# apple/ml-pgdvs

Hardware: AMD Instinct MI355X
Metric: novel-view frames/s at 1080p x 24 src frames; achieved HBM GB/s vs gfx950 peak (higher is better)
Workload: dtype f32

## Files before the change

### ml-pgdvs_amd/csrc/common.h

```cpp
#pragma once
#include <hip/hip_runtime.h>
#include <stdint.h>
#include <stdio.h>

#include "../../include/pgdvs_hip.h"

#define PGDVS_API extern "C" __attribute__((visibility("default")))

namespace pgdvs {

void set_error(const char *fmt, ...);

struct Options {
  int agg_ordered;
  int agg_stage;
  int gnt_fp32;
  int knn_no_tpq;
  int knn_stats;
  float raster_bound_density;
  int side_thread;
};
const char *last_error_text();
int option_int(const int &field);
float option_float(const float &field);
const Options &options();

inline hipStream_t as_stream(pgdvs_stream_t s) { return reinterpret_cast<hipStream_t>(s); }

inline int check_launch(const char *what) {
  hipError_t e = hipGetLastError();
  if (e != hipSuccess) {
    set_error("%s: %s", what, hipGetErrorString(e));
    return PGDVS_ERR_LAUNCH;
  }
  return PGDVS_OK;
}

bool prof_enabled();
void prof_begin(const char *name, hipStream_t s);
void prof_end(hipStream_t s);
struct ProfScope {
  hipStream_t s;
  bool on;
  ProfScope(const char *name, hipStream_t st) : s(st), on(prof_enabled()) {
    if (on) prof_begin(name, s);
  }
  ~ProfScope() {
    if (on) prof_end(s);
  }
};

#define PGDVS_LAUNCH(name, kernel, grid, block, lds, stream, ...)       \
  do {                                                                   \
    pgdvs::ProfScope _ps(name, stream);                                  \
    hipLaunchKernelGGL(kernel, grid, block, lds, stream, __VA_ARGS__);   \
  } while (0)

#define PGDVS_REQUIRE(cond, ...)      \
  do {                                \
    if (!(cond)) {                    \
      pgdvs::set_error(__VA_ARGS__);  \
      return PGDVS_ERR_INVALID;       \
    }                                 \
  } while (0)

constexpr int kWave = 64;

__global__ static void __launch_bounds__(256) fill_bytes_kernel(uint4 *__restrict__ p, int64_t n16, uint32_t v32) {
  const uint4 v = make_uint4(v32, v32, v32, v32);
  for (int64_t i = (int64_t)blockIdx.x * blockDim.x + threadIdx.x; i < n16; i += (int64_t)gridDim.x * blockDim.x) p[i] = v;
}

inline hipError_t fill_async(void *ptr, unsigned char byte, size_t nbytes, hipStream_t st) {
  if (nbytes < (1u << 20) || (reinterpret_cast<uintptr_t>(ptr) & 15) != 0) return hipMemsetAsync(ptr, byte, nbytes, st);
  const int64_t n16 = (int64_t)(nbytes / 16);
  const uint32_t v32 = 0x01010101u * byte;
  const unsigned grid = (unsigned)((n16 + 255) / 256 < 4096 ? (n16 + 255) / 256 : 4096);
  {
    ProfScope ps("fill_bytes", st);
    hipLaunchKernelGGL(fill_bytes_kernel, dim3(grid), dim3(256), 0, st, reinterpret_cast<uint4 *>(ptr), n16, v32);
  }
  const size_t tail = nbytes - (size_t)n16 * 16;
  if (tail) return hipMemsetAsync(static_cast<char *>(ptr) + (size_t)n16 * 16, byte, tail, st);
  return hipGetLastError();
}

inline int64_t cdiv(int64_t a, int64_t b) { return (a + b - 1) / b; }
inline int64_t align_up(int64_t a, int64_t b) { return cdiv(a, b) * b; }

struct Carver {
  char *base;
  int64_t off = 0;
  template <class T>
  T *take(int64_t bytes, int64_t align = 256) {
    T *p = reinterpret_cast<T *>(base + off);
    off += align_up(bytes, align);
    return p;
  }
};

struct CamBlock {
  float v[PGDVS_CAM_BLOCK];
};

__host__ __device__ inline int inv_f64(const double *a, double *out, int n) {
  double m[4][8];
  for (int i = 0; i < n; ++i) {
    for (int j = 0; j < n; ++j) {
      m[i][j] = a[i * n + j];
      m[i][n + j] = (i == j) ? 1.0 : 0.0;
    }
  }
  for (int c = 0; c < n; ++c) {
    int piv = c;
    double best = fabs(m[c][c]);
    for (int r = c + 1; r < n; ++r) {
      double v = fabs(m[r][c]);
      if (v > best) {
        best = v;
        piv = r;
      }
    }
    if (best == 0.0) return -1;
    if (piv != c) {
      for (int j = 0; j < 2 * n; ++j) {
        double t = m[c][j];
        m[c][j] = m[piv][j];
        m[piv][j] = t;
      }
    }
    double d = m[c][c];
    for (int j = 0; j < 2 * n; ++j) m[c][j] = m[c][j] / d;
    for (int r = 0; r < n; ++r) {
      if (r == c) continue;
      double f = m[r][c];
      if (f == 0.0) continue;
      for (int j = 0; j < 2 * n; ++j) m[r][j] = m[r][j] - f * m[c][j];
    }
  }
  for (int i = 0; i < n; ++i)
    for (int j = 0; j < n; ++j) out[i * n + j] = m[i][n + j];
  return 0;
}

__host__ __device__ inline int cam_block_from_flat(const float *flat_cam, float *blk) {
  const float *K = flat_cam + 2;
  const float *c2w = flat_cam + 18;
  double k3[9], k3i[9], c4[16], c4i[16];
  for (int i = 0; i < 3; ++i)
    for (int j = 0; j < 3; ++j) k3[i * 3 + j] = (double)K[i * 4 + j];
  for (int i = 0; i < 16; ++i) c4[i] = (double)c2w[i];
  int bad = 0;
  if (inv_f64(k3, k3i, 3) != 0) bad = 1;
  if (inv_f64(c4, c4i, 4) != 0) bad = 1;
  float kinv[9], w2c[16];
  for (int i = 0; i < 9; ++i) kinv[i] = bad ? __builtin_nanf("") : (float)k3i[i];
  for (int i = 0; i < 16; ++i) w2c[i] = bad ? __builtin_nanf("") : (float)c4i[i];
  for (int i = 0; i < 9; ++i) blk[PGDVS_CAM_KINV + i] = kinv[i];
  for (int i = 0; i < 3; ++i) {
    for (int j = 0; j < 3; ++j) {
      float s = c2w[i * 4 + 0] * kinv[0 * 3 + j];
      s = s + c2w[i * 4 + 1] * kinv[1 * 3 + j];
      s = s + c2w[i * 4 + 2] * kinv[2 * 3 + j];
      blk[PGDVS_CAM_M + i * 3 + j] = s;
      blk[PGDVS_CAM_R + i * 3 + j] = c2w[i * 4 + j];
    }
    blk[PGDVS_CAM_O + i] = c2w[i * 4 + 3];
// ... 54 lines not shown
```

### ml-pgdvs_amd/csrc/error.cpp

```cpp
#include <hip/hip_runtime.h>
#include <stdarg.h>
#include <string.h>

#include <map>
#include <mutex>
#include <string>
#include <vector>
#include <stdio.h>

#include <stdlib.h>

#include "common.h"

namespace pgdvs {
static thread_local char g_err[512] = "";

void set_error(const char *fmt, ...) {
  va_list ap;
  va_start(ap, fmt);
  vsnprintf(g_err, sizeof(g_err), fmt, ap);
  va_end(ap);
}

const char *last_error_text() { return g_err; }

struct ProfRec {
  const char *name;
  hipEvent_t a, b;
};
static std::mutex g_prof_mu;
static bool g_prof_on = false;
static std::vector<ProfRec> g_prof_recs;
static std::vector<hipEvent_t> g_prof_pool;
static thread_local ProfRec g_prof_cur;

bool prof_enabled() { return g_prof_on; }

static hipEvent_t prof_event() {
  std::lock_guard<std::mutex> lk(g_prof_mu);
  if (!g_prof_pool.empty()) {
    hipEvent_t e = g_prof_pool.back();
    g_prof_pool.pop_back();
    return e;
  }
  hipEvent_t e;
  (void)hipEventCreate(&e);
  return e;
}

void prof_begin(const char *name, hipStream_t s) {
  g_prof_cur.name = name;
  g_prof_cur.a = prof_event();
  g_prof_cur.b = prof_event();
  (void)hipEventRecord(g_prof_cur.a, s);
}

void prof_end(hipStream_t s) {
  (void)hipEventRecord(g_prof_cur.b, s);
  std::lock_guard<std::mutex> lk(g_prof_mu);
  g_prof_recs.push_back(g_prof_cur);
}
}

namespace pgdvs {
static Options options_from_env() {
  auto flag = [](const char *name) {
    const char *v = getenv(name);
    return v != nullptr && v[0] == '1' ? 1 : 0;
  };
  Options o;
  o.agg_ordered = flag("PGDVS_AGG_ORDERED");
  o.agg_stage = getenv("PGDVS_AGG_STAGE") != nullptr && getenv("PGDVS_AGG_STAGE")[0] == '0' ? 0 : 1;
  o.gnt_fp32 = flag("PGDVS_GNT_FP32");
  o.knn_no_tpq = flag("PGDVS_KNN_NO_TPQ");
  o.knn_stats = flag("PGDVS_KNN_STATS");
  const char *d = getenv("PGDVS_RASTER_BOUND_DENSITY");
  o.raster_bound_density = d != nullptr ? (float)atof(d) : 2.2f;
  o.side_thread = getenv("PGDVS_SIDE_THREAD") != nullptr && getenv("PGDVS_SIDE_THREAD")[0] == '0' ? 0 : 1;
  return o;
}
static Options g_options = options_from_env();
const Options &options() { return g_options; }
int option_int(const int &field) { return __atomic_load_n(&field, __ATOMIC_RELAXED); }
float option_float(const float &field) {
  float v;
  __atomic_load(&field, &v, __ATOMIC_RELAXED);
  return v;
}
struct OptionName {
  const char *name;
  int *i;
  float *f;
};
static const OptionName kOptionNames[] = {
    {"agg_ordered", &g_options.agg_ordered, nullptr},   {"agg_stage", &g_options.agg_stage, nullptr},
    {"gnt_fp32", &g_options.gnt_fp32, nullptr},
    {"knn_no_tpq", &g_options.knn_no_tpq, nullptr},     {"knn_stats", &g_options.knn_stats, nullptr},
    {"raster_bound_density", nullptr, &g_options.raster_bound_density},
    {"side_thread", &g_options.side_thread, nullptr},
};
}

extern "C" __attribute__((visibility("default"))) int pgdvs_option_set(const char *name, double value) {
  for (const auto &o : pgdvs::kOptionNames) {
    if (name != nullptr && strcmp(name, o.name) == 0) {
      if (o.i != nullptr) {
        __atomic_store_n(o.i, value != 0.0 ? 1 : 0, __ATOMIC_RELAXED);
      } else {
        float v = (float)value;
        __atomic_store(o.f, &v, __ATOMIC_RELAXED);
      }
      return PGDVS_OK;
    }
  }
  pgdvs::set_error("pgdvs_option_set: unknown option '%s'", name ? name : "(null)");
  return PGDVS_ERR_INVALID;
}

extern "C" __attribute__((visibility("default"))) double pgdvs_option_get(const char *name) {
  for (const auto &o : pgdvs::kOptionNames) {
    if (name != nullptr && strcmp(name, o.name) == 0)
      return o.i != nullptr ? (double)pgdvs::option_int(*o.i) : (double)pgdvs::option_float(*o.f);
  }
  return __builtin_nan("");
}

namespace pgdvs {
__global__ void prof_null_kernel() {}

static double prof_bracket_overhead_ms() {
  static double cached = -1.0;
  if (cached >= 0.0) return cached;
  hipEvent_t a, b;
  if (hipEventCreate(&a) != hipSuccess || hipEventCreate(&b) != hipSuccess) return 0.0;
  double best = 1e30;
  (void)hipDeviceSynchronize();
  for (int i = 0; i < 32; ++i) {
    (void)hipEventRecord(a, nullptr);
    prof_null_kernel<<<1, 64, 0, nullptr>>>();
    (void)hipEventRecord(b, nullptr);
    (void)hipEventSynchronize(b);
    float ms = 0.f;
    if (hipEventElapsedTime(&ms, a, b) == hipSuccess && ms > 0.f && ms < best) best = ms;
  }
  (void)hipEventDestroy(a);
  (void)hipEventDestroy(b);
  cached = best < 1e29 ? best : 0.0;
  return cached;
}
}

extern "C" __attribute__((visibility("default"))) double pgdvs_prof_overhead_ms(void) {
  return pgdvs::prof_bracket_overhead_ms();
}

extern "C" __attribute__((visibility("default"))) void pgdvs_prof_enable(int on) {
  std::lock_guard<std::mutex> lk(pgdvs::g_prof_mu);
  pgdvs::g_prof_on = on != 0;
}

extern "C" __attribute__((visibility("default"))) int pgdvs_prof_report(char *buf, int buf_len) {
  using namespace pgdvs;
  std::vector<ProfRec> recs;
  {
    std::lock_guard<std::mutex> lk(g_prof_mu);
    recs.swap(g_prof_recs);
  }
  std::map<std::string, std::pair<int, double>> agg;
  const double overhead = recs.empty() ? 0.0 : prof_bracket_overhead_ms();
  for (auto &r : recs) {
    (void)hipEventSynchronize(r.b);
    float ms = 0.f;
    (void)hipEventElapsedTime(&ms, r.a, r.b);
    auto &e = agg[r.name];
    e.first += 1;
    e.second += ms > overhead ? ms - overhead : 0.0;
    std::lock_guard<std::mutex> lk(g_prof_mu);
    g_prof_pool.push_back(r.a);
    g_prof_pool.push_back(r.b);
  }
  std::string out;
  for (auto &kv : agg) {
    char line[256];
    snprintf(line, sizeof(line), "%s %d %.6f\n", kv.first.c_str(), kv.second.first, kv.second.second);
    out += line;
  }
  if (buf && buf_len > 0) {
    strncpy(buf, out.c_str(), (size_t)buf_len - 1);
    buf[buf_len - 1] = 0;
  }
  return (int)agg.size();
}

extern "C" __attribute__((visibility("default"))) const char *pgdvs_last_error(void) {
  return pgdvs::g_err;
}
extern "C" __attribute__((visibility("default"))) int pgdvs_abi_version(void) { return 1; }
extern "C" __attribute__((visibility("default"))) const char *pgdvs_build_arch(void) {
  return "gfx950";
}
```

### ml-pgdvs_amd/csrc/static_agg.hip

```cpp
#include <cmath>
#include <vector>

#include "common.h"
#include "wave.h"

namespace pgdvs {

struct ProjF64 {
  double K3[9];
  double w2c[16];
  int affine;
  int ksparse;
  double M[12];
  double tol_scale;
  int screen;
  float M32[12];
  float e32[3];
  int screen32;
};

__device__ __forceinline__ double refined_rcp(double b) {
  double r = __builtin_amdgcn_rcp(b);
  double e = __builtin_fma(-b, r, 1.0);
  r = __builtin_fma(r, e, r);
  e = __builtin_fma(-b, r, 1.0);
  return __builtin_fma(r, e, r);
}

__device__ __forceinline__ bool trunc_div_in_range(double a, double b, double r, int hi, int &out) {
  double q = a * r;
  double f = floor(q);
  double dist = fmin(q - f, (f + 1.0) - q);
  if (!(dist > fabs(q) * 1e-13 + 1e-290)) q = a / b;
  if (!(q >= 0.0 && q <= (double)hi)) return false;
  out = (int)q;
  return true;
}

constexpr int kProjChunk = 10;
struct ProjChunk {
  ProjF64 p[kProjChunk];
};
static_assert(sizeof(ProjChunk) + 64 <= 4096, "agg_params_kernel's arguments");

struct PushConsts;
__global__ void agg_params_kernel(ProjChunk c, ProjF64 *__restrict__ dst, float *__restrict__ pc32, int first, int n, float q_hi) {
  const int words = (int)(sizeof(ProjF64) / 4);
  for (int k = threadIdx.x; k < n * words; k += blockDim.x)
    reinterpret_cast<uint32_t *>(dst + first)[k] = reinterpret_cast<const uint32_t *>(&c.p[0])[k];
  for (int k = threadIdx.x; k < n * 16; k += blockDim.x) {
    const ProjF64 &pj = c.p[k >> 4];
    const int j = k & 15;
    float v = 0.0f;
    if (j < 12) {
      v = pj.M32[j];
    } else if (!pj.screen32) {
      v = j < 15 ? INFINITY : 0.0f;
    } else if (j == 12) {
      const double e01 = pj.e32[0] > pj.e32[1] ? (double)pj.e32[0] : (double)pj.e32[1];
      v = (float)((e01 + ((double)q_hi + 1.0) * (double)pj.e32[2]) * 1.001 * 1.000001);
    } else if (j == 13) {
      v = (float)(((double)q_hi * 2.6e-7 + 1e-7) * 1.000001);
    } else if (j == 14) {
      v = (float)((0.125 - ((double)q_hi * 2.6e-7 + 1e-7) * 1.000001) * 0.999999);
    }
    pc32[(size_t)(first + (k >> 4)) * 16 + j] = v;
  }
}

struct ByteStamp {
  uint8_t *occ_all;
  int64_t P;
  unsigned *stat;
  __device__ __forceinline__ void operator()(int f, int q) const { (occ_all + (int64_t)f * P)[(unsigned)q] = 1; }
};
template <class Stamp>
__device__ __attribute__((noinline)) void mark_reference_order(const ProjF64 *__restrict__ pj, double x, double y,
                                                               double z, int H, int W, int f, const Stamp &stamp) {
  double vc[4];
#pragma unroll
  for (int k = 0; k < 3; ++k) {
    double s = pj->w2c[k * 4 + 0] * x;
    s = s + pj->w2c[k * 4 + 1] * y;
    s = s + pj->w2c[k * 4 + 2] * z;
    s = s + pj->w2c[k * 4 + 3];
    vc[k] = s;
  }
  double cx = vc[0], cy = vc[1], cz = vc[2];
  if (!pj->affine) {
    double s = pj->w2c[12] * x;
    s = s + pj->w2c[13] * y;
    s = s + pj->w2c[14] * z;
    s = s + pj->w2c[15];
    cx = vc[0] / s;
    cy = vc[1] / s;
    cz = vc[2] / s;
  }
  double pp[3];
  if (pj->ksparse) {
    pp[0] = pj->K3[0] * cx + pj->K3[2] * cz;
    pp[1] = pj->K3[4] * cy + pj->K3[5] * cz;
    pp[2] = cz;
  } else {
#pragma unroll
    for (int k = 0; k < 3; ++k) {
      double s = pj->K3[k * 3 + 0] * cx;
      s = s + pj->K3[k * 3 + 1] * cy;
      s = s + pj->K3[k * 3 + 2] * cz;
      pp[k] = s;
    }
  }
  int row, col;
  const double rz = refined_rcp(pp[2]);
  if (!trunc_div_in_range(pp[1], pp[2], rz, H - 1, row)) return;
  if (!trunc_div_in_range(pp[0], pp[2], rz, W - 1, col)) return;
  stamp(f, row * W + col);
}

template <class Stamp>
__device__ __attribute__((noinline)) void mark_fp64(const ProjF64 *__restrict__ pj, float xf, float yf, float zf, int H,
                                                    int W, int f, const Stamp &stamp) {
  const double x = (double)xf, y = (double)yf, z = (double)zf;
  if (pj->screen) {
    const double *M = pj->M;
    const double amax = fmax(fmax(fabs(x), fabs(y)), fmax(fabs(z), 1.0));
    const double s0 = __builtin_fma(M[0], x, __builtin_fma(M[1], y, __builtin_fma(M[2], z, M[3])));
    const double s1 = __builtin_fma(M[4], x, __builtin_fma(M[5], y, __builtin_fma(M[6], z, M[7])));
    const double s2 = __builtin_fma(M[8], x, __builtin_fma(M[9], y, __builtin_fma(M[10], z, M[11])));
    const double r = refined_rcp(s2);
    const double qx = s0 * r, qy = s1 * r;
    const double tol = pj->tol_scale * amax * fabs(r);
    const double fx = floor(qx), fy = floor(qy);
    const double dx = fmin(qx - fx, (fx + 1.0) - qx), dy = fmin(qy - fy, (fy + 1.0) - qy);
    if (dx > tol * (1.0 + fabs(qx)) && dy > tol * (1.0 + fabs(qy))) {
      if (qy >= 0.0 && qy <= (double)(H - 1) && qx >= 0.0 && qx <= (double)(W - 1)) stamp(f, (int)qy * W + (int)qx);
      return;
    }
  }
  atomicAdd(stamp.stat, 1u);
  mark_reference_order(pj, x, y, z, H, W, f, stamp);
}

typedef float f2v __attribute__((ext_vector_type(2)));
struct PushConsts {
  float M[12];
  float e[3];
  float pad;
};
static_assert(sizeof(PushConsts) == 64, "PushConsts");

struct AppendSrc {
  const float *depth;
  const float *rgb;
  float *cloud;
  float *xyz;
  int P, W;
};
struct f3 { float x, y, z; };

__device__ __forceinline__ f3 append_row(const AppendSrc &a, const CamBlock &cam, int p, int64_t pos, bool write,
                                         float d_in = __builtin_nanf(""), float *d_out = nullptr, const f3 *c_in = nullptr) {
  int r, col;
  if (a.P < (1 << 24)) {
    r = (int)(((float)p + 0.5f) * (1.0f / (float)a.W));
    col = p - r * a.W;
    if (col < 0) {
      --r;
      col += a.W;
    } else if (col >= a.W) {
      ++r;
      col -= a.W;
    }
  } else {
    r = p / a.W;
    col = p - r * a.W;
  }
  const float u = (float)col, v = (float)r;
  const float d = d_in == d_in ? d_in : a.depth[p];
  if (d_out) *d_out = d;
  float X[3];
#pragma unroll
  for (int ax = 0; ax < 3; ++ax) {
    float dir = cam.v[PGDVS_CAM_M + ax * 3 + 0] * u;
    dir = dir + cam.v[PGDVS_CAM_M + ax * 3 + 1] * v;
    dir = dir + cam.v[PGDVS_CAM_M + ax * 3 + 2];
    X[ax] = cam.v[PGDVS_CAM_O + ax] + dir * d;
  }
  f3 xq;
  xq.x = X[0];
  xq.y = X[1];
  xq.z = X[2];
  if (write) {
    const f3 c = c_in ? *c_in : *reinterpret_cast<const f3 *>(a.rgb + (size_t)p * 3);
    float2 *o = reinterpret_cast<float2 *>(a.cloud + pos * 6);
    o[0] = make_float2(X[0], X[1]);
    o[1] = make_float2(X[2], c.x);
    o[2] = make_float2(c.y, c.z);
    *reinterpret_cast<f3 *>(a.xyz + pos * 3) = xq;
  }
  return xq;
}

constexpr int kSelThreads = 512;
constexpr int kSelItems = 16;
constexpr int kSelTile = kSelThreads * kSelItems;
constexpr int kPushThreads = 256;
constexpr int kPushQueue = 1024;
constexpr int kPushQueueSmall = 512;
constexpr int kPushMaxFpg = 32;

template <class Stamp, class Rec>
__device__ __forceinline__ unsigned screen_frames(const Rec &rec, const int fa, const int fb,
                                                  const bool live, float x, float y, float z, const float wm1,
                                                  const float hm1, const int W, const Stamp &stamp) {
  if (!live) x = y = z = __builtin_nanf("");
  const float amax = fmaxf(fmaxf(fabsf(x), fabsf(y)), fmaxf(fabsf(z), 1.0f));
  unsigned dmask = 0;
  auto frame = [&](const int f, const PushConsts &c) {
    const float *M = c.M;
    const f2v p0 = {M[0], M[1]}, p1 = {M[2], M[3]}, p2 = {M[4], M[5]}, p3 = {M[6], M[7]};
    const f2v xx = {x, x}, yy = {y, y}, zz = {z, z};
    const f2v s01 = __builtin_elementwise_fma(p0, xx, __builtin_elementwise_fma(p1, yy, __builtin_elementwise_fma(p2, zz, p3)));
    const float s0 = s01.x, s1 = s01.y;
    const float s2 = __builtin_fmaf(M[8], x, __builtin_fmaf(M[9], y, __builtin_fmaf(M[10], z, M[11])));
    const float r = __builtin_amdgcn_rcpf(s2);
    const float qx = s0 * r, qy = s1 * r;
    const float u = c.e[0] * (fabsf(r) * amax);
    const float gx = __builtin_amdgcn_fractf(qx), gy = __builtin_amdgcn_fractf(qy);
    const float dx = fminf(gx, 1.0f - gx), dy = fminf(gy, 1.0f - gy);
    const bool sure = (__builtin_fmaf(qx + qy, 0.0f, u) < c.e[2]) & (fabsf(s2) < 0x1p100f);
    const bool clear = fminf(dx, dy) - u > c.e[1];
    const float mi = fminf(fminf(qx, wm1 - qx), fminf(qy, hm1 - qy));
    if (sure & clear & (mi >= 0.0f)) stamp(f, (int)qy * W + (int)qx);
    dmask |= ((sure & (clear | (mi < -0.5f))) ? 0u : 1u) << (f - fa);
  };
  PushConsts ca = rec(fa);
  for (int f = fa; f < fb; f += 2) {
    const PushConsts cb = rec(f + 1);
    frame(f, ca);
    if (f + 1 < fb) {
      ca = rec(f + 2);
      frame(f + 1, cb);
    }
  }
  return live ? dmask : 0u;
}

constexpr int kAggStatWords = 65;
template <int kQueue, int kThreads, class Stamp>
__device__ __forceinline__ void queue_doubtful(uint4 *s_q, int *s_qn, const unsigned dmask, const float x, const float y,
                                               const float z, const int fa, const bool last,
                                               const ProjF64 *__restrict__ proj, const int H, const int W, const Stamp &stamp) {
  if (dmask != 0) {
    const int slot = atomicAdd(s_qn, 1);
    if (slot < kQueue) {
      s_q[slot] = make_uint4(__float_as_uint(x), __float_as_uint(y), __float_as_uint(z), dmask);
    } else {
      atomicAdd(stamp.stat + 1 + (blockIdx.x & 63), 1u);
      for (unsigned m = dmask; m; m &= m - 1) {
        const int f = fa + __builtin_ctz(m);
        mark_fp64(proj + f, x, y, z, H, W, f, stamp);
      }
    }
  }
  __syncthreads();
  const int qn = *s_qn < kQueue ? *s_qn : kQueue;
  __syncthreads();
  if (last || qn + kThreads > kQueue) {
    if (threadIdx.x == 0) s_qn[1] += qn;
    for (int e = threadIdx.x; e < qn; e += kThreads) {
      const uint4 q = s_q[e];
      const float px = __uint_as_float(q.x), py = __uint_as_float(q.y), pz = __uint_as_float(q.z);
      for (unsigned m = q.w; m; m &= m - 1) {
        const int f = fa + __builtin_ctz(m);
        mark_fp64(proj + f, px, py, pz, H, W, f, stamp);
      }
    }
    __syncthreads();
    if (threadIdx.x == 0) {
      *s_qn = 0;
      if (last && s_qn[1] > 0) {
        atomicAdd(stamp.stat + 1 + (blockIdx.x & 63), (unsigned)s_qn[1]);
        s_qn[1] = 0;
      }
    }
    __syncthreads();
  }
}

template <int kQueue>
__global__ void __launch_bounds__(kPushThreads)
agg_push_kernel(const float *__restrict__ xyz, const int64_t *__restrict__ cnts, int src,
                const ProjF64 *__restrict__ proj, const PushConsts *__restrict__ pc, int f_lo, int f_hi, int fpg, int H, int W,
                uint8_t *__restrict__ occ_all, const int32_t *__restrict__ sel_pix, AppendSrc app, CamBlock cam,
                unsigned *__restrict__ stat) {
  __shared__ uint4 s_q[kQueue];
  __shared__ int s_qn[2];
  const int64_t begin = cnts[src], end = cnts[src + 1];
  if (begin >= end) return;
  const ByteStamp stamp{occ_all, (int64_t)H * W, stat};
  const float wm1 = (float)(W - 1), hm1 = (float)(H - 1);
  if (threadIdx.x == 0) s_qn[0] = s_qn[1] = 0;
  __syncthreads();
  bool first_iter = true;
  for (int fa = f_lo + (int)blockIdx.y * fpg; fa < f_hi || (first_iter && sel_pix != nullptr && blockIdx.y == 0);
       fa += (int)gridDim.y * fpg, first_iter = false) {
  const int fb = fa >= f_hi ? fa : (fa + fpg < f_hi ? fa + fpg : f_hi);
  const int64_t n_chunks = (end - begin + kPushThreads - 1) / kPushThreads;
  const int64_t per_xcd = (n_chunks + 7) / 8;
  const int64_t c_lo = (int64_t)(blockIdx.x & 7) * per_xcd;
  const int64_t c_hi = c_lo + per_xcd < n_chunks ? c_lo + per_xcd : n_chunks;
  const int64_t c_step = gridDim.x >> 3 ? gridDim.x >> 3 : 1;
  for (int64_t ch = c_lo + (int64_t)(blockIdx.x >> 3); ch < c_hi; ch += c_step) {
    const int64_t i = begin + ch * kPushThreads + threadIdx.x;
    const bool live = i < end;
    float x = 0.f, y = 0.f, z = 0.f;
    if (live && sel_pix != nullptr) {
      const f3 X = append_row(app, cam, sel_pix[i - begin], i, blockIdx.y == 0 && first_iter);
      x = X.x;
      y = X.y;
      z = X.z;
    } else if (live) {
      x = xyz[i * 3 + 0];
      y = xyz[i * 3 + 1];
      z = xyz[i * 3 + 2];
    }
    unsigned dmask = 0;
    if (fa < fb) dmask = screen_frames([pc](const int f) { return pc[f]; }, fa, fb, live, x, y, z, wm1, hm1, W, stamp);
    queue_doubtful<kQueue, kPushThreads>(s_q, s_qn, dmask, x, y, z, fa, ch + c_step >= c_hi, proj, H, W, stamp);
  }
  }
}


constexpr int kBitTileWords = kSelTile / 32;
constexpr int kStepThreads = 256;
constexpr int kStepPx = 16;
constexpr int kStepChunkPx = 128;
constexpr int kStepChunks = kStepThreads * kStepPx / kStepChunkPx;

__device__ __forceinline__ int64_t step_chunk_of(const int b, const int r, const int gx) {
  const int L = gx >> 3, xcd = b & 7, l = b >> 3;
  const int j = r * L + l;
  return ((int64_t)(j / kStepChunks) * 8 + xcd) * kStepChunks + (j % kStepChunks);
}
__device__ __forceinline__ void step_owner_of(const int64_t g, const int gx, int &b, int &r) {
  const int L = gx >> 3;
  const int64_t stripe = g / kStepChunks;
  const int xcd = (int)(stripe & 7);
  const int j = (int)(stripe >> 3) * kStepChunks + (int)(g % kStepChunks);
  r = j / L;
  b = (j - r * L) * 8 + xcd;
}

constexpr unsigned kSelSpinLimit = 1u << 22;

__device__ __forceinline__ unsigned long long sel_desc(int tag, int status, long long v) {
  return ((unsigned long long)tag << 48) | ((unsigned long long)status << 46) | (unsigned long long)v;
}

struct SelArgs {
  const uint8_t *dyn_mask;
  const uint8_t *occ;
  const float *depth;
  const float *rgb;
  float *cloud;
  float *xyz;
  int64_t *cnts;
  unsigned long long *desc;
  int32_t *ticket;
  int32_t *error;
  int32_t *sel_pix;
  int64_t capacity;
  int frame, P, W, tiles;
};

__device__ __forceinline__ unsigned sel_flags16(const SelArgs &a, int base) {
  unsigned flags = 0;
  if (base + kSelItems <= a.P && ((reinterpret_cast<uintptr_t>(a.dyn_mask + base) & 15) == 0)) {
    const uint4 m = *reinterpret_cast<const uint4 *>(a.dyn_mask + base);
    const unsigned mw[4] = {m.x, m.y, m.z, m.w};
#pragma unroll
    for (int k = 0; k < 16; ++k) flags |= (((mw[k >> 2] >> ((k & 3) * 8)) & 0xffu) == 0u ? 1u : 0u) << k;
    if (a.frame > 0 && ((reinterpret_cast<uintptr_t>(a.occ + base) & 15) == 0)) {
      const uint4 o = *reinterpret_cast<const uint4 *>(a.occ + base);
      const unsigned ow[4] = {o.x, o.y, o.z, o.w};
      unsigned stamped = 0;
#pragma unroll
      for (int k = 0; k < 16; ++k) stamped |= (((ow[k >> 2] >> ((k & 3) * 8)) & 0xffu) != 0u ? 1u : 0u) << k;
      flags &= ~stamped;
    } else if (a.frame > 0) {
      unsigned stamped = 0;
#pragma unroll
      for (int k = 0; k < 16; ++k) stamped |= (a.occ[base + k] != 0 ? 1u : 0u) << k;
      flags &= ~stamped;
    }
  } else {
    for (int k = 0; k < kSelItems; ++k) {
      const int p = base + k;
      if (p >= a.P) break;
      bool st = a.dyn_mask[p] == 0;
      if (a.frame > 0) st = st && a.occ[p] == 0;
      flags |= (st ? 1u : 0u) << k;
    }
  }
  return flags;
}

__device__ __forceinline__ unsigned zero_bytes16(const uint4 v) {
  const unsigned w[4] = {v.x, v.y, v.z, v.w};
  unsigned bits = 0;
#pragma unroll
  for (int k = 0; k < 4; ++k) {
    const unsigned nz = ((((w[k] & 0x7f7f7f7fu) + 0x7f7f7f7fu) | w[k]) >> 7) & 0x01010101u;
    bits |= ((nz * 0x10204080u) >> 28) << (4 * k);
  }
  return ~bits & 0xffffu;
}

__global__ void __launch_bounds__(kSelThreads) agg_select_kernel(SelArgs a, CamBlock cam) {
  __shared__ int s_tile;
  __shared__ int wave_sums[kSelThreads / kWave];
  __shared__ long long s_excl;
  __shared__ uint16_t s_list[kSelTile];
  const int tid = threadIdx.x, lane = tid & 63, wave = tid >> 6;
  if (tid == 0) s_tile = atomicAdd(&a.ticket[a.frame], 1);
  __syncthreads();
  const int tile = s_tile;
  const int base = tile * kSelTile + tid * kSelItems;
  const unsigned flags = base < a.P ? sel_flags16(a, base) : 0u;
  const int c = __popc(flags);
  int total;
  const int excl = block_excl_scan<kSelThreads / kWave>(c, wave_sums, total);
  const int tag = a.frame + 1;
  if (tid == 0)
    __hip_atomic_store(&a.desc[tile], sel_desc(tag, 1, total), __ATOMIC_RELAXED, __HIP_MEMORY_SCOPE_AGENT);
  if (total == 0 && tile != a.tiles - 1) return;
  long long part = 0;
  for (int j = tid; j < tile; j += kSelThreads) {
    unsigned spins = 0;
    unsigned long long d;
    while (true) {
      d = __hip_atomic_load(&a.desc[j], __ATOMIC_RELAXED, __HIP_MEMORY_SCOPE_AGENT);
      if ((int)(d >> 48) == tag) break;
      if (++spins > kSelSpinLimit) {
        atomicExch(a.error, 1);
        break;
      }
      __builtin_amdgcn_s_sleep(1);
    }
    part += (long long)(d & ((1ull << 46) - 1));
  }
  part = wave_sum_down(part);
  __shared__ long long wave_part[kSelThreads / kWave];
  if (lane == 0) wave_part[wave] = part;
  __syncthreads();
  if (tid == 0) {
    long long e = 0;
#pragma unroll
    for (int w = 0; w < kSelThreads / kWave; ++w) e += wave_part[w];
    s_excl = e;
  }
  __syncthreads();
  const int64_t cloud_base = a.cnts[a.frame];
  if (tile == a.tiles - 1 && tid == 0) {
    int64_t n = cloud_base + s_excl + total;
    n = n > a.capacity ? a.capacity : n;
    a.cnts[a.frame + 1] = n;
  }
  if (total == 0) return;
  {
    int slot = excl;
    unsigned f = flags;
    while (f) {
      const int k = __builtin_ctz(f);
      f &= f - 1;
      s_list[slot++] = (uint16_t)(tid * kSelItems + k);
    }
  }
  __syncthreads();
  const int64_t pos0 = cloud_base + s_excl;
  const int tile_px = tile * kSelTile;
  if (a.sel_pix != nullptr) {
// ... 291 lines not shown
                                 void *zero_extra = nullptr, int64_t zero_extra_bytes = 0);

PGDVS_API int pgdvs_static_aggregate(const float *rgbs, const float *depths,
                                     const uint8_t *dyn_masks, const double *K3s_host,
                                     const double *c2ws_host, int S, int H, int W, float *out,
                                     int64_t capacity, int64_t *count_out, void *workspace,
                                     int64_t workspace_bytes, pgdvs_stream_t stream) {
  return static_aggregate_impl(rgbs, depths, dyn_masks, K3s_host, c2ws_host, S, H, W, out, nullptr, capacity, count_out,
                               workspace, workspace_bytes, stream);
}

PGDVS_API int pgdvs_static_aggregate_packed(const float *rgbs, const float *depths,
                                            const uint8_t *dyn_masks, const double *K3s_host,
                                            const double *c2ws_host, int S, int H, int W, float *out, float *xyz_out,
                                            int64_t capacity, int64_t *count_out, void *workspace,
                                            int64_t workspace_bytes, pgdvs_stream_t stream) {
  PGDVS_REQUIRE(xyz_out, "pgdvs_static_aggregate_packed: null pointer");
  return static_aggregate_impl(rgbs, depths, dyn_masks, K3s_host, c2ws_host, S, H, W, out, xyz_out, capacity, count_out,
                               workspace, workspace_bytes, stream);
}

namespace pgdvs {
int static_aggregate_for_view(const float *rgbs, const float *depths, const uint8_t *dyn_masks, const double *K3s_host,
                              const double *c2ws_host, int S, int H, int W, float *out, float *xyz_out, int64_t capacity,
                              int64_t *count_out, void *workspace, int64_t workspace_bytes, pgdvs_stream_t stream,
                              bool params_cached, void *zero_extra, int64_t zero_extra_bytes) {
  return static_aggregate_impl(rgbs, depths, dyn_masks, K3s_host, c2ws_host, S, H, W, out, xyz_out, capacity, count_out, workspace,
                               workspace_bytes, stream, params_cached, zero_extra, zero_extra_bytes);
}
}

static int static_aggregate_impl(const float *rgbs, const float *depths, const uint8_t *dyn_masks,
                                 const double *K3s_host, const double *c2ws_host, int S, int H, int W, float *out,
                                 float *xyz_out, int64_t capacity, int64_t *count_out, void *workspace,
                                 int64_t workspace_bytes, pgdvs_stream_t stream, bool params_cached, void *zero_extra,
                                 int64_t zero_extra_bytes) {
  PGDVS_REQUIRE(rgbs && depths && dyn_masks && K3s_host && c2ws_host && out && count_out,
                "pgdvs_static_aggregate: null pointer");
  PGDVS_REQUIRE(S > 0 && S < 65535 && H > 0 && W > 0 && (int64_t)H * W < (1ll << 31) && capacity > 0 &&
                    capacity < (1ll << 45),
                "pgdvs_static_aggregate: bad shape");
  AggWs ws = agg_ws_layout(workspace, S, H, W, capacity);
  if (!workspace || workspace_bytes < ws.total_bytes) {
    set_error("pgdvs_static_aggregate: workspace too small");
    return PGDVS_ERR_WORKSPACE;
  }
  if (xyz_out) ws.xyz = xyz_out;
  hipStream_t st = as_stream(stream);
  const int64_t P = (int64_t)H * W;
  hipError_t e = fill_async(ws.state, 0, (size_t)(reinterpret_cast<char *>(ws.sel) - ws.state) + (size_t)S * (size_t)ws.Wd * 4, st);
  if (e != hipSuccess) {
    set_error("static_aggregate memset: %s", hipGetErrorString(e));
    return PGDVS_ERR_LAUNCH;
  }
  std::vector<CamBlock> cams((size_t)S);
  {
    ProjChunk chunk;
    for (int i = 0; i < S; ++i) {
      const double *K3 = K3s_host + (size_t)i * 9;
      const double *c2w = c2ws_host + (size_t)i * 16;
      ProjF64 &pj = chunk.p[i % kProjChunk];
      for (int k = 0; k < 9; ++k) pj.K3[k] = K3[k];
      if (inv_f64(c2w, pj.w2c, 4) != 0) {
        set_error("pgdvs_static_aggregate: singular c2w for frame %d", i);
        return PGDVS_ERR_INVALID;
      }
      pj.affine = pj.w2c[12] == 0.0 && pj.w2c[13] == 0.0 && pj.w2c[14] == 0.0 && pj.w2c[15] == 1.0;
      pj.ksparse = K3[1] == 0.0 && K3[3] == 0.0 && K3[6] == 0.0 && K3[7] == 0.0 && K3[8] == 1.0;
      {
        double rmax = 0.0;
        bool finite = true;
        for (int r = 0; r < 3; ++r) {
          double rowsum = 0.0;
          for (int c = 0; c < 4; ++c) {
            double m = 0.0, a = 0.0;
            for (int k = 0; k < 3; ++k) {
              m += K3[r * 3 + k] * pj.w2c[k * 4 + c];
              a += fabs(K3[r * 3 + k]) * fabs(pj.w2c[k * 4 + c]);
            }
            pj.M[r * 4 + c] = m;
            rowsum += a;
            finite = finite && std::isfinite(m) && std::isfinite(a);
          }
          rmax = rowsum > rmax ? rowsum : rmax;
        }
        pj.tol_scale = 64.0 * 1.1102230246251565e-16 * rmax;
        pj.screen = pj.affine && finite && rmax > 0.0;
        bool ok32 = pj.screen != 0;
        for (int k = 0; k < 12; ++k) {
          const int pos = k < 8 ? (k & 3) * 2 + (k >> 2) : k;
          pj.M32[pos] = (float)pj.M[k];
          ok32 = ok32 && std::isfinite(pj.M32[pos]);
        }
        for (int r = 0; r < 3; ++r) {
          double rowsum = 0.0;
          for (int c = 0; c < 4; ++c) rowsum += fabs(pj.M[r * 4 + c]);
          const double e = (4.5 * 5.9604644775390625e-08 * rowsum + pj.tol_scale) * 1.000001;
          pj.e32[r] = nextafterf((float)e, INFINITY);
          ok32 = ok32 && std::isfinite(pj.e32[r]);
        }
        pj.screen32 = ok32 ? 1 : 0;
      }
      float flat[34];
      flat[0] = (float)H;
      flat[1] = (float)W;
      for (int r = 0; r < 4; ++r)
        for (int c = 0; c < 4; ++c)
          flat[2 + r * 4 + c] = (r < 3 && c < 3) ? (float)K3[r * 3 + c] : (r == c ? 1.0f : 0.0f);
      for (int k = 0; k < 16; ++k) flat[18 + k] = (float)c2w[k];
      if (cam_block_from_flat(flat, cams[(size_t)i].v) != 0) {
        set_error("pgdvs_static_aggregate: singular intrinsics for frame %d", i);
        return PGDVS_ERR_INVALID;
      }
      if (!params_cached && (i % kProjChunk == kProjChunk - 1 || i == S - 1)) {
        const int first = i - i % kProjChunk, cnt = i % kProjChunk + 1;
        PGDVS_LAUNCH("agg_params", agg_params_kernel, dim3(1), dim3(256), 0, st, chunk, ws.proj, reinterpret_cast<float *>(ws.pc32), first,
                     cnt, (float)((W > H ? W : H) + 1));
      }
    }
  }
  const int tiles = (int)cdiv(P, kSelTile);
  const bool bit_chain = option_int(options().agg_ordered) == 0 && S > 1;
  auto select = [&](int i) {
    SelArgs a;
    a.dyn_mask = dyn_masks + (size_t)i * P;
    a.occ = ws.occ + (size_t)i * (size_t)P;
    a.depth = depths + (size_t)i * P;
    a.rgb = rgbs + (size_t)i * P * 3;
    a.cloud = out;
    a.xyz = ws.xyz;
    a.cnts = ws.cnts;
    a.desc = ws.desc;
    a.ticket = ws.ticket;
    a.error = ws.error;
    a.sel_pix = i > 0 ? ws.sel_pix : nullptr;
    a.capacity = capacity;
    a.frame = i;
    a.P = (int)P;
    a.W = W;
    a.tiles = tiles;
    PGDVS_LAUNCH("agg_select", agg_select_kernel, dim3(tiles), dim3(kSelThreads), 0, st, a, cams[(size_t)i]);
  };
  auto frame_src = [&](int i) {
    AppendSrc app;
    app.depth = depths + (size_t)i * P;
    app.rgb = rgbs + (size_t)i * P * 3;
    app.cloud = out;
    app.xyz = ws.xyz;
    app.P = (int)P;
    app.W = W;
    return app;
  };
  const int fpg = 12;
  auto push = [&](int i) {
    const int fpg_i = i == 0 ? fpg : (fpg > 4 ? 4 : fpg);
    const int groups = i + 1 < S ? (int)cdiv(S - 1 - i, fpg_i) : 1;
    const int64_t want = i == 0 ? cdiv(P, kPushThreads) : (cdiv(P, 8 * kPushThreads) < 256 ? cdiv(P, 8 * kPushThreads) : 256);
    const unsigned gx = (unsigned)(want < 1024 ? (want > 8 ? (want + 7) / 8 * 8 : 8) : 1024);
    if (i == 0) {
      PGDVS_LAUNCH("agg_push0", agg_push_kernel<kPushQueue>, dim3(gx, (unsigned)groups), dim3(kPushThreads), 0, st,
                   (const float *)ws.xyz, (const int64_t *)ws.cnts, i, (const ProjF64 *)ws.proj, (const PushConsts *)ws.pc32, i + 1, S, fpg_i, H, W,
                   ws.occ,
                   (const int32_t *)nullptr, frame_src(i), cams[(size_t)i], ws.stat);
    } else {
      PGDVS_LAUNCH("agg_push", agg_push_kernel<kPushQueueSmall>, dim3(gx, (unsigned)groups), dim3(kPushThreads), 0, st,
                   (const float *)ws.xyz, (const int64_t *)ws.cnts, i, (const ProjF64 *)ws.proj, (const PushConsts *)ws.pc32, i + 1, S, fpg_i, H, W,
                   ws.occ,
                   (const int32_t *)ws.sel_pix, frame_src(i), cams[(size_t)i], ws.stat);
    }
  };
  if (!bit_chain) {
    if (zero_extra != nullptr && zero_extra_bytes > 0) (void)hipMemsetAsync(zero_extra, 0, (size_t)zero_extra_bytes, st);
    for (int i = 0; i < S; ++i) {
      select(i);
      if (i + 1 < S || i > 0) push(i);
    }
    PGDVS_LAUNCH("agg_finalize", agg_finalize_kernel, dim3(1), dim3(64), 0, st, (const int64_t *)ws.cnts,
                 (const int32_t *)ws.error, (const int64_t *)nullptr, S, capacity, count_out);
    return check_launch("static_aggregate");
  }
  if (!params_cached) {
    CamChunk chunk;
    const int per = (int)(sizeof(chunk.c) / sizeof(chunk.c[0]));
    for (int i = 1; i < S; ++i) {
      chunk.c[(i - 1) % per] = cams[(size_t)i];
      if ((i - 1) % per == per - 1 || i == S - 1) {
        const int cnt = (i - 1) % per + 1;
        PGDVS_LAUNCH("agg_cams", agg_cams_kernel, dim3(1), dim3(256), 0, st, chunk, ws.cams, i - cnt + 1, cnt);
      }
    }
  }
  select(0);
  push(0);
  RowStage stage;
  stage.rows = option_int(options().agg_stage) != 0 ? ws.stage_rows : nullptr;
  stage.cst = ws.stage_cst;
  stage.gx = ws.step_gx;
  {
    const unsigned gx = (unsigned)ws.step_gx;
    const int sfpg = kPushMaxFpg;
    for (int i = 1; i < S; ++i) {
      SelArgs a;
      a.dyn_mask = dyn_masks + (size_t)i * P;
      a.occ = ws.occ + (size_t)i * (size_t)P;
      a.frame = i;
      a.P = (int)P;
      a.W = W;
      const unsigned gy = i + 1 < S ? (unsigned)cdiv(S - 1 - i, sfpg) : 1u;
      PGDVS_LAUNCH("agg_step", agg_step_kernel<kPushQueueSmall>, dim3(gx, gy), dim3(kStepThreads), 0, st, a, ws.occ,
                   reinterpret_cast<uint16_t *>(ws.sel), ws.Wd, i, (const ProjF64 *)ws.proj, (const PushConsts *)ws.pc32, S, sfpg, H, W,
                   frame_src(i), cams[(size_t)i], ws.stat, stage);
    }
  }
  PGDVS_LAUNCH("agg_count", agg_count_kernel, dim3((unsigned)tiles, (unsigned)(S - 1)), dim3(kBitTileWords), 0, st,
               (const uint32_t *)ws.sel, ws.Wd, tiles, ws.tile_cnt);
  {
    RowsArgs ra;
    ra.depths = depths;
    ra.rgbs = rgbs;
    ra.cloud = out;
    ra.xyz = ws.xyz;
    ra.capacity = capacity;
    ra.P = (int)P;
    ra.W = W;
    PGDVS_LAUNCH("agg_rows", agg_rows_kernel, dim3((unsigned)tiles, (unsigned)(S - 1)), dim3(kBitTileWords), 0, st,
                 (const uint32_t *)ws.sel, ws.Wd, tiles, (const int32_t *)ws.tile_cnt, (const int64_t *)ws.cnts,
                 (const CamBlock *)ws.cams, ra, stage, stage.rows != nullptr ? S - 1 : 0, reinterpret_cast<uint4 *>(zero_extra),
                 (int)(zero_extra_bytes / 16), (const int32_t *)ws.error, count_out);
  }
  return check_launch("static_aggregate");
}
```

Baseline: 1325.

## Add specialized frame-0 push kernel with inlined fp64 fallback and vector constant loads

Adds a dedicated agg_push0 kernel for the bit-chain path. It screens points against all frames using 16-wide vector loads of per-frame constants, writes occupancy bytes directly, and inlines the fp64 fallback instead of calling noinline functions. The kernel is templated on points per thread, currently set to 1, and the old generic kernel stays reachable behind an env flag. The aim is to cut call overhead and constant-load cost in the dominant first-frame push, at the risk of higher register pressure from inlining the fp64 path.

```diff
diff --git a/ml-pgdvs_amd/csrc/common.h b/ml-pgdvs_amd/csrc/common.h
--- a/ml-pgdvs_amd/csrc/common.h
+++ b/ml-pgdvs_amd/csrc/common.h
@@ -13,6 +13,7 @@
 
 struct Options {
   int agg_ordered;
+  int agg_push_single;
   int agg_stage;
   int gnt_fp32;
   int knn_no_tpq;
diff --git a/ml-pgdvs_amd/csrc/error.cpp b/ml-pgdvs_amd/csrc/error.cpp
--- a/ml-pgdvs_amd/csrc/error.cpp
+++ b/ml-pgdvs_amd/csrc/error.cpp
@@ -70,6 +70,7 @@
   };
   Options o;
   o.agg_ordered = flag("PGDVS_AGG_ORDERED");
+  o.agg_push_single = flag("PGDVS_AGG_PUSH_SINGLE");
   o.agg_stage = getenv("PGDVS_AGG_STAGE") != nullptr && getenv("PGDVS_AGG_STAGE")[0] == '0' ? 0 : 1;
   o.gnt_fp32 = flag("PGDVS_GNT_FP32");
   o.knn_no_tpq = flag("PGDVS_KNN_NO_TPQ");
@@ -94,6 +95,7 @@
 };
 static const OptionName kOptionNames[] = {
     {"agg_ordered", &g_options.agg_ordered, nullptr},   {"agg_stage", &g_options.agg_stage, nullptr},
+    {"agg_push_single", &g_options.agg_push_single, nullptr},
     {"gnt_fp32", &g_options.gnt_fp32, nullptr},
     {"knn_no_tpq", &g_options.knn_no_tpq, nullptr},     {"knn_stats", &g_options.knn_stats, nullptr},
     {"raster_bound_density", nullptr, &g_options.raster_bound_density},
diff --git a/ml-pgdvs_amd/csrc/static_agg.hip b/ml-pgdvs_amd/csrc/static_agg.hip
--- a/ml-pgdvs_amd/csrc/static_agg.hip
+++ b/ml-pgdvs_amd/csrc/static_agg.hip
@@ -75,8 +75,8 @@
   __device__ __forceinline__ void operator()(int f, int q) const { (occ_all + (int64_t)f * P)[(unsigned)q] = 1; }
 };
 template <class Stamp>
-__device__ __attribute__((noinline)) void mark_reference_order(const ProjF64 *__restrict__ pj, double x, double y,
-                                                               double z, int H, int W, int f, const Stamp &stamp) {
+__device__ __forceinline__ void mark_reference_order_body(const ProjF64 *__restrict__ pj, double x, double y, double z, int H,
+                                                          int W, int f, const Stamp &stamp) {
   double vc[4];
 #pragma unroll
   for (int k = 0; k < 3; ++k) {
@@ -116,10 +116,15 @@
   if (!trunc_div_in_range(pp[0], pp[2], rz, W - 1, col)) return;
   stamp(f, row * W + col);
 }
-
 template <class Stamp>
-__device__ __attribute__((noinline)) void mark_fp64(const ProjF64 *__restrict__ pj, float xf, float yf, float zf, int H,
-                                                    int W, int f, const Stamp &stamp) {
+__device__ __attribute__((noinline)) void mark_reference_order(const ProjF64 *__restrict__ pj, double x, double y,
+                                                               double z, int H, int W, int f, const Stamp &stamp) {
+  mark_reference_order_body(pj, x, y, z, H, W, f, stamp);
+}
+
+template <bool kInline, class Stamp>
+__device__ __forceinline__ void mark_fp64_body(const ProjF64 *__restrict__ pj, float xf, float yf, float zf, int H, int W, int f,
+                                               const Stamp &stamp) {
   const double x = (double)xf, y = (double)yf, z = (double)zf;
   if (pj->screen) {
     const double *M = pj->M;
@@ -138,7 +143,15 @@
     }
   }
   atomicAdd(stamp.stat, 1u);
-  mark_reference_order(pj, x, y, z, H, W, f, stamp);
+  if (kInline)
+    mark_reference_order_body(pj, x, y, z, H, W, f, stamp);
+  else
+    mark_reference_order(pj, x, y, z, H, W, f, stamp);
+}
+template <class Stamp>
+__device__ __attribute__((noinline)) void mark_fp64(const ProjF64 *__restrict__ pj, float xf, float yf, float zf, int H,
+                                                    int W, int f, const Stamp &stamp) {
+  mark_fp64_body<false>(pj, xf, yf, zf, H, W, f, stamp);
 }
 
 typedef float f2v __attribute__((ext_vector_type(2)));
@@ -209,6 +222,30 @@
 constexpr int kPushQueueSmall = 512;
 constexpr int kPushMaxFpg = 32;
 
+struct Screened {
+  float qx, qy;
+  bool hit, decided;
+};
+__device__ __forceinline__ Screened screen_point(const PushConsts &c, const float x, const float y, const float z, const float amax,
+                                                 const float wm1, const float hm1) {
+  const float *M = c.M;
+  const f2v p0 = {M[0], M[1]}, p1 = {M[2], M[3]}, p2 = {M[4], M[5]}, p3 = {M[6], M[7]};
+  const f2v xx = {x, x}, yy = {y, y}, zz = {z, z};
+  const f2v s01 = __builtin_elementwise_fma(p0, xx, __builtin_elementwise_fma(p1, yy, __builtin_elementwise_fma(p2, zz, p3)));
+  const float s0 = s01.x, s1 = s01.y;
+  const float s2 = __builtin_fmaf(M[8], x, __builtin_fmaf(M[9], y, __builtin_fmaf(M[10], z, M[11])));
+  const float r = __builtin_amdgcn_rcpf(s2);
+  const float qx = s0 * r, qy = s1 * r;
+  const float u = c.e[0] * (fabsf(r) * amax);
+  const float gx = __builtin_amdgcn_fractf(qx), gy = __builtin_amdgcn_fractf(qy);
+  const float dx = fminf(gx, 1.0f - gx), dy = fminf(gy, 1.0f - gy);
+  const bool sure = (__builtin_fmaf(qx + qy, 0.0f, u) < c.e[2]) & (fabsf(s2) < 0x1p100f);
+  const bool clear = fminf(dx, dy) - u > c.e[1];
+  const float mi = fminf(fminf(qx, wm1 - qx), fminf(qy, hm1 - qy));
+  const bool hit = sure & clear & (mi >= 0.0f), decided = sure & (clear | (mi < -0.5f));
+  return Screened{qx, qy, hit, decided};
+}
+
 template <class Stamp, class Rec>
 __device__ __forceinline__ unsigned screen_frames(const Rec &rec, const int fa, const int fb,
                                                   const bool live, float x, float y, float z, const float wm1,
@@ -217,22 +254,9 @@
   const float amax = fmaxf(fmaxf(fabsf(x), fabsf(y)), fmaxf(fabsf(z), 1.0f));
   unsigned dmask = 0;
   auto frame = [&](const int f, const PushConsts &c) {
-    const float *M = c.M;
-    const f2v p0 = {M[0], M[1]}, p1 = {M[2], M[3]}, p2 = {M[4], M[5]}, p3 = {M[6], M[7]};
-    const f2v xx = {x, x}, yy = {y, y}, zz = {z, z};
-    const f2v s01 = __builtin_elementwise_fma(p0, xx, __builtin_elementwise_fma(p1, yy, __builtin_elementwise_fma(p2, zz, p3)));
-    const float s0 = s01.x, s1 = s01.y;
-    const float s2 = __builtin_fmaf(M[8], x, __builtin_fmaf(M[9], y, __builtin_fmaf(M[10], z, M[11])));
-    const float r = __builtin_amdgcn_rcpf(s2);
-    const float qx = s0 * r, qy = s1 * r;
-    const float u = c.e[0] * (fabsf(r) * amax);
-    const float gx = __builtin_amdgcn_fractf(qx), gy = __builtin_amdgcn_fractf(qy);
-    const float dx = fminf(gx, 1.0f - gx), dy = fminf(gy, 1.0f - gy);
-    const bool sure = (__builtin_fmaf(qx + qy, 0.0f, u) < c.e[2]) & (fabsf(s2) < 0x1p100f);
-    const bool clear = fminf(dx, dy) - u > c.e[1];
-    const float mi = fminf(fminf(qx, wm1 - qx), fminf(qy, hm1 - qy));
-    if (sure & clear & (mi >= 0.0f)) stamp(f, (int)qy * W + (int)qx);
-    dmask |= ((sure & (clear | (mi < -0.5f))) ? 0u : 1u) << (f - fa);
+    const Screened s = screen_point(c, x, y, z, amax, wm1, hm1);
+    if (s.hit) stamp(f, (int)s.qy * W + (int)s.qx);
+    dmask |= (s.decided ? 0u : 1u) << (f - fa);
   };
   PushConsts ca = rec(fa);
   for (int f = fa; f < fb; f += 2) {
@@ -246,34 +270,86 @@
   return live ? dmask : 0u;
 }
 
+typedef float f16v __attribute__((ext_vector_type(16)));
+__device__ __forceinline__ PushConsts load_consts(const PushConsts *__restrict__ p) {
+  const f16v v = *reinterpret_cast<const f16v *>(p);
+  PushConsts c;
+#pragma unroll
+  for (int j = 0; j < 12; ++j) c.M[j] = v[j];
+  c.e[0] = v[12];
+  c.e[1] = v[13];
+  c.e[2] = v[14];
+  c.pad = v[15];
+  return c;
+}
+template <int kPts>
+__device__ __forceinline__ void screen_frames_pts(const PushConsts *__restrict__ pc, const int fa, const int fb,
+                                                  const bool (&live)[kPts], float (&x)[kPts], float (&y)[kPts], float (&z)[kPts],
+                                                  const float wm1, const float hm1, const int W, uint8_t *__restrict__ occ_all,
+                                                  const int64_t P, unsigned (&dmask)[kPts]) {
+  float amax[kPts];
+#pragma unroll
+  for (int u = 0; u < kPts; ++u) {
+    if (!live[u]) x[u] = y[u] = z[u] = __builtin_nanf("");
+    amax[u] = fmaxf(fmaxf(fabsf(x[u]), fabsf(y[u])), fmaxf(fabsf(z[u]), 1.0f));
+    dmask[u] = 0;
+  }
+  auto frame = [&](const int k, const PushConsts &c, uint8_t *__restrict__ occ_f) {
+    Screened s[kPts];
+#pragma unroll
+    for (int u = 0; u < kPts; ++u) {
+      s[u] = screen_point(c, x[u], y[u], z[u], amax[u], wm1, hm1);
+      dmask[u] |= (s[u].decided ? 1u : 0u) << k;
+    }
+#pragma unroll
+    for (int u = 0; u < kPts; ++u)
+      if (s[u].hit) occ_f[(unsigned)((int)s[u].qy * W + (int)s[u].qx)] = 1;
+  };
+  const PushConsts *__restrict__ p = pc + fa;
+  uint8_t *__restrict__ occ = occ_all + (int64_t)fa * P;
+  const int n = fb - fa;
+  for (int k = 0; k < n; ++k, ++p, occ += P) frame(k, load_consts(p), occ);
+#pragma unroll
+  for (int u = 0; u < kPts; ++u) dmask[u] = live[u] ? ~dmask[u] & (0xffffffffu >> (32 - n)) : 0u;
+}
+
 constexpr int kAggStatWords = 65;
-template <int kQueue, int kThreads, class Stamp>
-__device__ __forceinline__ void queue_doubtful(uint4 *s_q, int *s_qn, const unsigned dmask, const float x, const float y,
-                                               const float z, const int fa, const bool last,
-                                               const ProjF64 *__restrict__ proj, const int H, const int W, const Stamp &stamp) {
-  if (dmask != 0) {
-    const int slot = atomicAdd(s_qn, 1);
-    if (slot < kQueue) {
-      s_q[slot] = make_uint4(__float_as_uint(x), __float_as_uint(y), __float_as_uint(z), dmask);
-    } else {
-      atomicAdd(stamp.stat + 1 + (blockIdx.x & 63), 1u);
-      for (unsigned m = dmask; m; m &= m - 1) {
-        const int f = fa + __builtin_ctz(m);
-        mark_fp64(proj + f, x, y, z, H, W, f, stamp);
+template <int kQueue, int kThreads, int kPts, bool kInline, class Stamp>
+__device__ __forceinline__ void queue_doubtful_pts(uint4 *s_q, int *s_qn, const unsigned (&dmask)[kPts], const float (&x)[kPts],
+                                                   const float (&y)[kPts], const float (&z)[kPts], const int fa, const bool last,
+                                                   const ProjF64 *__restrict__ proj, const int H, const int W, const Stamp &stamp) {
+  auto mark = [&](const float px, const float py, const float pz, const int f) {
+    if (kInline)
+      mark_fp64_body<true>(proj + f, px, py, pz, H, W, f, stamp);
+    else
+      mark_fp64(proj + f, px, py, pz, H, W, f, stamp);
+  };
+#pragma unroll
+  for (int u = 0; u < kPts; ++u) {
+    if (dmask[u] != 0) {
+      const int slot = atomicAdd(s_qn, 1);
+      if (slot < kQueue) {
+        s_q[slot] = make_uint4(__float_as_uint(x[u]), __float_as_uint(y[u]), __float_as_uint(z[u]), dmask[u]);
+      } else {
+        atomicAdd(stamp.stat + 1 + (blockIdx.x & 63), 1u);
+        for (unsigned m = dmask[u]; m; m &= m - 1) {
+          const int f = fa + __builtin_ctz(m);
+          mark(x[u], y[u], z[u], f);
+        }
       }
     }
   }
   __syncthreads();
   const int qn = *s_qn < kQueue ? *s_qn : kQueue;
   __syncthreads();
-  if (last || qn + kThreads > kQueue) {
+  if (last || qn + kPts * kThreads > kQueue) {
     if (threadIdx.x == 0) s_qn[1] += qn;
     for (int e = threadIdx.x; e < qn; e += kThreads) {
       const uint4 q = s_q[e];
       const float px = __uint_as_float(q.x), py = __uint_as_float(q.y), pz = __uint_as_float(q.z);
       for (unsigned m = q.w; m; m &= m - 1) {
         const int f = fa + __builtin_ctz(m);
-        mark_fp64(proj + f, px, py, pz, H, W, f, stamp);
+        mark(px, py, pz, f);
       }
     }
     __syncthreads();
@@ -286,6 +362,14 @@
     }
     __syncthreads();
   }
+}
+template <int kQueue, int kThreads, class Stamp>
+__device__ __forceinline__ void queue_doubtful(uint4 *s_q, int *s_qn, const unsigned dmask, const float x, const float y,
+                                               const float z, const int fa, const bool last,
+                                               const ProjF64 *__restrict__ proj, const int H, const int W, const Stamp &stamp) {
+  const unsigned dm[1] = {dmask};
+  const float xs[1] = {x}, ys[1] = {y}, zs[1] = {z};
+  queue_doubtful_pts<kQueue, kThreads, 1, false>(s_q, s_qn, dm, xs, ys, zs, fa, last, proj, H, W, stamp);
 }
 
 template <int kQueue>
@@ -329,6 +413,49 @@
     if (fa < fb) dmask = screen_frames([pc](const int f) { return pc[f]; }, fa, fb, live, x, y, z, wm1, hm1, W, stamp);
     queue_doubtful<kQueue, kPushThreads>(s_q, s_qn, dmask, x, y, z, fa, ch + c_step >= c_hi, proj, H, W, stamp);
   }
+  }
+}
+
+constexpr int kPushPts = 1;
+template <int kQueue, int kPts>
+__global__ void __launch_bounds__(kPushThreads)
+agg_push0_kernel(const float *__restrict__ xyz, const int64_t *__restrict__ cnts, int src, const ProjF64 *__restrict__ proj,
+                 const PushConsts *__restrict__ pc, int f_lo, int f_hi, int fpg, int H, int W, uint8_t *__restrict__ occ_all,
+                 unsigned *__restrict__ stat) {
+  __shared__ uint4 s_q[kQueue];
+  __shared__ int s_qn[2];
+  const int64_t begin = cnts[src], end = cnts[src + 1];
+  if (begin >= end) return;
+  const ByteStamp stamp{occ_all, (int64_t)H * W, stat};
+  const float wm1 = (float)(W - 1), hm1 = (float)(H - 1);
+  if (threadIdx.x == 0) s_qn[0] = s_qn[1] = 0;
+  __syncthreads();
+  constexpr int kChunk = kPts * kPushThreads;
+  const int64_t n_chunks = (end - begin + kChunk - 1) / kChunk;
+  const int64_t per_xcd = (n_chunks + 7) / 8;
+  const int64_t c_lo = (int64_t)(blockIdx.x & 7) * per_xcd;
+  const int64_t c_hi = c_lo + per_xcd < n_chunks ? c_lo + per_xcd : n_chunks;
+  const int64_t c_step = gridDim.x >> 3 ? gridDim.x >> 3 : 1;
+  for (int fa = f_lo + (int)blockIdx.y * fpg; fa < f_hi; fa += (int)gridDim.y * fpg) {
+    const int fb = fa + fpg < f_hi ? fa + fpg : f_hi;
+    for (int64_t ch = c_lo + (int64_t)(blockIdx.x >> 3); ch < c_hi; ch += c_step) {
+      bool live[kPts];
+      float x[kPts], y[kPts], z[kPts];
+      unsigned dmask[kPts];
+#pragma unroll
+      for (int u = 0; u < kPts; ++u) {
+        const int64_t i = begin + ch * kChunk + u * kPushThreads + threadIdx.x;
+        live[u] = i < end;
+        x[u] = y[u] = z[u] = 0.f;
+        if (live[u]) {
+          x[u] = xyz[i * 3 + 0];
+          y[u] = xyz[i * 3 + 1];
+          z[u] = xyz[i * 3 + 2];
+        }
+      }
+      screen_frames_pts<kPts>(pc, fa, fb, live, x, y, z, wm1, hm1, W, occ_all, stamp.P, dmask);
+      queue_doubtful_pts<kQueue, kPushThreads, kPts, true>(s_q, s_qn, dmask, x, y, z, fa, ch + c_step >= c_hi, proj, H, W, stamp);
+    }
   }
 }
 
@@ -926,12 +1053,19 @@
     return app;
   };
   const int fpg = 12;
+  const bool push0_pts = bit_chain && option_int(options().agg_push_single) == 0;
   auto push = [&](int i) {
     const int fpg_i = i == 0 ? fpg : (fpg > 4 ? 4 : fpg);
     const int groups = i + 1 < S ? (int)cdiv(S - 1 - i, fpg_i) : 1;
     const int64_t want = i == 0 ? cdiv(P, kPushThreads) : (cdiv(P, 8 * kPushThreads) < 256 ? cdiv(P, 8 * kPushThreads) : 256);
     const unsigned gx = (unsigned)(want < 1024 ? (want > 8 ? (want + 7) / 8 * 8 : 8) : 1024);
-    if (i == 0) {
+    if (i == 0 && push0_pts) {
+      const int64_t want0 = cdiv(P, kPushPts * kPushThreads);
+      const unsigned gx0 = (unsigned)(want0 < 1024 ? (want0 > 8 ? (want0 + 7) / 8 * 8 : 8) : 1024);
+      PGDVS_LAUNCH("agg_push0", (agg_push0_kernel<kPushQueue, kPushPts>), dim3(gx0, (unsigned)groups), dim3(kPushThreads), 0, st,
+                   (const float *)ws.xyz, (const int64_t *)ws.cnts, i, (const ProjF64 *)ws.proj, (const PushConsts *)ws.pc32, i + 1, S, fpg_i, H, W,
+                   ws.occ, ws.stat);
+    } else if (i == 0) {
       PGDVS_LAUNCH("agg_push0", agg_push_kernel<kPushQueue>, dim3(gx, (unsigned)groups), dim3(kPushThreads), 0, st,
                    (const float *)ws.xyz, (const int64_t *)ws.cnts, i, (const ProjF64 *)ws.proj, (const PushConsts *)ws.pc32, i + 1, S, fpg_i, H, W,
                    ws.occ,
```

Result: faster. 1353, median of 6 (+2.2%).
